# joedownard/skill-chaining-with-graphs

Measured on AMD Instinct MI355X. Metric: env-steps/sec (whole node), 65 536 parallel Pinball envs at 1/2/4/8 MI355X, higher is better.
Workload: dtype f32

## Files before the change

### skill-chaining-with-graphs_amd/csrc/scg_kernels.hip

```cpp
#include "scg_device.hpp"
#include "../../include/scg_abi.h"
#include <cstdio>
#include <cstdlib>
#include <cstring>
#include <cmath>
#include <mutex>
#include <new>
#include <type_traits>
#include <vector>

using namespace scg;
typedef float f4v __attribute__((ext_vector_type(4)));
typedef unsigned u4v __attribute__((ext_vector_type(4)));

#include "scg_eval.hpp"
#include "scg_step_kernel.hpp"
#include "scg_rollout_kernel.hpp"
#include "scg_trial_kernel.hpp"
#include "scg_order.hpp"
#include "scg_collect_kernels.hpp"
#include "scg_reduce_kernel.hpp"
#include "scg_apply_kernels.hpp"
#include "scg_aux_kernels.hpp"

__attribute__((visibility("hidden"))) hipError_t launch_rollout_record(const RolloutRecArgs &A, int grid, hipStream_t s);
__attribute__((visibility("hidden"))) hipError_t launch_trial_record(const TrialRecArgs &A, int grid, hipStream_t s);
__attribute__((visibility("hidden"))) hipError_t launch_rollout_interrupt(const RolloutIntArgs &A, int grid, hipStream_t s);
__attribute__((visibility("hidden"))) hipError_t launch_rollout_interrupt_record(const RolloutIntRecArgs &A, int grid, hipStream_t s);

struct scg_ctx {
    scg_config cfg;
    int n_vf;
    int nblk;
    int n_cu;
    bool have_map;
    MapScalars ms;
    float *d_edges, *d_starts, *d_scale;
    uint64_t *d_cellmask;
    int32_t *d_perm, *d_hist;
    int32_t *d_collect_rows;
    int32_t *d_frontier_rows;
    uint32_t arm_bits;
    const uint8_t *arm_prev;
    const int32_t *arm_count;
    int32_t arm_L;
    bool arm_rows_ready;
    unsigned long long *d_fit_part;
    uint32_t *h_async;
    uint32_t *d_async;
    int32_t *d_fail;
    double fit_timeout_s;
    float4 *d_outrec;
    float4 *d_qalt;
    int32_t *d_invperm;
    int32_t *d_hist2[2];
    int hist_parity;
    bool hist_dirty;
    bool order_valid;
    const int32_t *order_ids;
    uint32_t parents;
    uint32_t gest;
    int32_t *gest_succ;
    float *ring_x, *ring_y;
    uint8_t *events;
    int32_t *ev_len;
    int32_t ring_len;
    unsigned long long *d_stamps;
    float *d_slabs;
    int32_t *d_cnts;
    float *d_G;
    int32_t *d_nk;
    float *G_out;
    int32_t *nk_out;
    float *nkf_out;
    bool prof_on;
    int prof_every;
    long long prof_seen;
    std::vector<hipEvent_t> *prof_ev;
    size_t prof_used;
    char *peer_region;
    size_t peer_bytes, peer_op_stride;
    hipIpcMemHandle_t peer_handle;
    int peer_n, peer_rank;
    char *peer_base[PEER_MAX];
    bool peer_mapped[PEER_MAX];
    uint32_t peer_e;
    int32_t *d_peer_go;
    double peer_timeout_s;
    char err[256];
};

static std::mutex g_peer_mu;
static std::vector<std::pair<hipIpcMemHandle_t, char *>> g_peer_regions;

static thread_local char g_err[256] = "";

#define SCG_HIP(ctx, call)                                                                     \
    do {                                                                                       \
        hipError_t e_ = (call);                                                                \
        if (e_ != hipSuccess) {                                                                \
            snprintf((ctx) ? (ctx)->err : g_err, 256, "%s failed: %s", #call, hipGetErrorString(e_)); \
            return SCG_ERR_HIP;                                                                \
        }                                                                                      \
    } while (0)

static int fail(scg_ctx *ctx, int code, const char *msg) {
    snprintf(ctx ? ctx->err : g_err, 256, "%s", msg);
    return code;
}

static int fail_in(scg_ctx *c, int code, const char *fn, const char *why) {
    char msg[256];
    snprintf(msg, sizeof(msg), "%s: %s", fn, why);
    return fail(c, code, msg);
}

static bool pow2(int x) { return x > 0 && !(x & (x - 1)); }
static bool bad_window(int32_t l_pos, int32_t l_neg) {
    return l_pos < 0 || l_neg < 0 || (int64_t)l_pos + l_neg < 1 || (int64_t)l_pos + l_neg > INT32_MAX;
}

static int decode_async(uint32_t word, char *buf, size_t n) {
    if (word == 0) { if (buf && n) buf[0] = 0; return SCG_OK; }
    if (buf && n) {
        if (word & SCG_ASYNC_STEP_HANDOFF)
            snprintf(buf, n, "an earlier scg_step gave up inside a workgroup: a bounded hand-off poll between its wavefront subsets ran "
                     "out (a logic error or a hung wavefront); the block's partial gradients were dropped and the step's outputs for "
                     "its envs are unspecified — restore the state. scg_clear_async_error() re-arms the context");
        else if (word & SCG_ASYNC_PEER_TIMEOUT)
            snprintf(buf, n, "an earlier scg_peer_exchange_apply gave up: the peer wait ran out (a peer rank did not publish its "
                     "operand within the peer timeout: stopped, hung or out of step); the weights were left unchanged. "
                     "scg_clear_async_error() re-arms the context");
        else if (word & SCG_ASYNC_FIT_TIMEOUT)
            snprintf(buf, n, "an earlier scg_fit_initiation gave up (problem mask 0x%x): its workgroups did not become "
                     "co-resident within the fit timeout (card shared with other work?); the affected classifier rows were "
                     "left unchanged. scg_clear_async_error() re-arms the context", (word >> 8) & 0xffffu);
        else
            snprintf(buf, n, "unknown asynchronous device status 0x%x", word);
    }
    return SCG_ERR_ASYNC;
}
static int async_pending(scg_ctx *c);
#define SCG_CHECK_ASYNC(c) do { if (async_pending(c)) return SCG_ERR_ASYNC; } while (0)

struct DeviceGuard {
    int prev = -1;
    bool ok = true;
    explicit DeviceGuard(int dev) {
        int cur = -1;
        if (hipGetDevice(&cur) != hipSuccess) { ok = false; return; }
        if (cur != dev) {
            if (hipSetDevice(dev) != hipSuccess) { ok = false; return; }
            prev = cur;
        }
    }
    ~DeviceGuard() { if (prev >= 0) (void)hipSetDevice(prev); }
    DeviceGuard(const DeviceGuard &) = delete;
    DeviceGuard &operator=(const DeviceGuard &) = delete;
};
#define SCG_ON_DEVICE(c, what)                                                                   \
    DeviceGuard dev_guard_((c)->cfg.device);                                                     \
    if (!dev_guard_.ok) return fail((c), SCG_ERR_HIP, what ": cannot make the context's device current")

static int async_pending(scg_ctx *c) {
    if (!c || !c->h_async) return 0;
    const uint32_t w = *reinterpret_cast<volatile uint32_t *>(c->h_async);
    if (w == 0) return 0;
    decode_async(w, c->err, sizeof(c->err));
    return 1;
}

extern "C" {

int scg_abi_version(void) { return SCG_ABI_VERSION; }

int scg_decode_async_word(uint32_t word, char *buf, int32_t buf_len) {
    return decode_async(word, buf, buf_len > 0 ? (size_t)buf_len : 0);
}

int scg_async_status(scg_ctx *c, void *stream, int32_t synchronize, uint32_t *word_out) {
    if (!c) return fail(nullptr, SCG_ERR_INVALID, "scg_async_status: null ctx");
    if (synchronize) {
        SCG_ON_DEVICE(c, "scg_async_status");
        SCG_HIP(c, hipStreamSynchronize(reinterpret_cast<hipStream_t>(stream)));
    }
    const uint32_t w = c->h_async ? *reinterpret_cast<volatile uint32_t *>(c->h_async) : 0u;
    if (word_out) *word_out = w;
    return decode_async(w, c->err, sizeof(c->err));
}

int scg_clear_async_error(scg_ctx *c) {
    if (!c) return fail(nullptr, SCG_ERR_INVALID, "scg_clear_async_error: null ctx");
    if (c->h_async) *reinterpret_cast<volatile uint32_t *>(c->h_async) = 0u;
    if (c->d_fail) {
        DeviceGuard g(c->cfg.device);
        if (g.ok) (void)hipMemset(c->d_fail, 0, sizeof(int32_t));
    }
    c->order_valid = false; c->hist_dirty = true; c->arm_rows_ready = false;
    return SCG_OK;
}

static int set_timeout(scg_ctx *c, const char *fn, double scg_ctx::*field, double seconds) {
    if (!c) return fail_in(nullptr, SCG_ERR_INVALID, fn, "null ctx");
    if (!(seconds >= 0.0) || seconds > 3600.0) return fail_in(c, SCG_ERR_INVALID, fn, "seconds must be in [0, 3600]");
    c->*field = seconds;
    return SCG_OK;
}

int scg_set_fit_timeout(scg_ctx *c, double seconds) { return set_timeout(c, "scg_set_fit_timeout", &scg_ctx::fit_timeout_s, seconds); }

int scg_set_peer_timeout(scg_ctx *c, double seconds) { return set_timeout(c, "scg_set_peer_timeout", &scg_ctx::peer_timeout_s, seconds); }

int scg_debug_raise_async(scg_ctx *c, uint32_t word) {
    if (!c || !c->h_async) return fail(c, SCG_ERR_INVALID, "scg_debug_raise_async: null ctx");
    *reinterpret_cast<volatile uint32_t *>(c->h_async) |= word;
    return SCG_OK;
}

int scg_block_envs(void) { return BLOCK_ENVS; }

const char *scg_strerror(int status) {
    switch (status) {
        case SCG_OK: return "ok";
        case SCG_ERR_INVALID: return "invalid argument";
        case SCG_ERR_NO_DEVICE: return "no usable HIP device";
        case SCG_ERR_HIP: return "HIP runtime error";
        case SCG_ERR_STATE: return "call order / state error";
        case SCG_ERR_ASYNC: return "an earlier launch failed on the device";
        default: return "unknown status";
    }
}

const char *scg_last_error(const scg_ctx *ctx) { return ctx ? ctx->err : g_err; }

static size_t hist_bytes(const scg_ctx *c) { return (size_t)((c->cfg.n_envs + 255) / 256) * HSTRIDE * sizeof(int32_t); }

struct CtxAlloc { void **ptr; size_t bytes; bool zero; };
static std::vector<CtxAlloc> ctx_allocs(scg_ctx *c) {
    auto P = [](auto **p) { return reinterpret_cast<void **>(p); };
    const size_t w = (size_t)c->n_vf * NACT * NF * sizeof(float), npos = (size_t)c->nblk * BLOCK_ENVS;
    const size_t rows = (size_t)(c->cfg.n_envs + COL_ROW - 1) / COL_ROW + 1;
    return {
        {P(&c->d_slabs), (size_t)c->nblk * w, false},
        {P(&c->d_cnts), (size_t)c->nblk * c->n_vf * sizeof(int32_t), true},
        {P(&c->d_G), w, true},
        {P(&c->d_nk), MAX_VF * sizeof(int32_t), true},
        {P(&c->d_edges), MAX_EDGES * 8 * sizeof(float), false},
        {P(&c->d_scale), NF * sizeof(float), false},
        {P(&c->d_perm), npos * sizeof(int32_t), false},
        {P(&c->d_hist), hist_bytes(c), false},
        {P(&c->d_collect_rows), rows * sizeof(int32_t), false},
        {P(&c->d_frontier_rows), MAX_VF * rows * sizeof(int32_t), false},
        {P(&c->d_fit_part), (size_t)FIT_BATCH * 2 * FIT_G * 8 * sizeof(unsigned long long), false},
        {P(&c->d_fail), sizeof(int32_t), true},
        {P(&c->d_outrec), npos * OREC * sizeof(float4), false},
        {P(&c->d_qalt), npos * 2 * sizeof(float4), false},
        {P(&c->d_invperm), npos * sizeof(int32_t), false},
        {P(&c->d_hist2[0]), hist_bytes(c), true},
        {P(&c->d_hist2[1]), hist_bytes(c), true},
        {P(&c->d_cellmask), (size_t)CELL_G * CELL_G * 4 * sizeof(uint64_t), false},
    };
}

#ifdef SCG_REDUCE_STAMPS
static size_t reduce_stamp_bytes(const scg_ctx *c) {
    const int nrow = (c->cfg.n_envs + 255) / 256, sy = (nrow + RED_NCOL - 1) / RED_NCOL;
    return (size_t)RED_NCOL * (c->n_vf + sy) * RED_STAMP_SLOTS * sizeof(unsigned long long);
}
#endif

int scg_create(scg_ctx **out, const scg_config *cfg) {
    if (!out || !cfg) return fail(nullptr, SCG_ERR_INVALID, "scg_create: null argument");
    *out = nullptr;
    if (cfg->n_envs < 1) return fail(nullptr, SCG_ERR_INVALID, "scg_create: n_envs must be >= 1");
    if (cfg->n_options < 0 || cfg->n_options > SCG_MAX_OPTIONS)
        return fail(nullptr, SCG_ERR_INVALID, "scg_create: n_options out of range [0,5]");
    if (cfg->update_count_floor < 0) return fail(nullptr, SCG_ERR_INVALID, "scg_create: update_count_floor must be >= 0");
    if (cfg->reoffer_period != 0 && !pow2(cfg->reoffer_period))
        return fail(nullptr, SCG_ERR_INVALID, "scg_create: reoffer_period must be a power of two (or 0)");
    if (cfg->fourier_order != SCG_FOURIER_ORDER)
        return fail(nullptr, SCG_ERR_INVALID, "scg_create: only Fourier order 5 is built");
    int ndev = 0;
    if (hipGetDeviceCount(&ndev) != hipSuccess || ndev < 1)
        return fail(nullptr, SCG_ERR_NO_DEVICE, "scg_create: no HIP device visible");
    if (cfg->device < 0 || cfg->device >= ndev)
        return fail(nullptr, SCG_ERR_INVALID, "scg_create: device ordinal out of range");
    scg_ctx *c = new (std::nothrow) scg_ctx();
    if (!c) return fail(nullptr, SCG_ERR_INVALID, "scg_create: out of host memory");
    memset(c, 0, sizeof(*c));
    c->cfg = *cfg;
    c->n_vf = cfg->n_options + 1;
    c->nblk = (cfg->n_envs + BLOCK_ENVS - 1) / BLOCK_ENVS;
    if (hipDeviceGetAttribute(&c->n_cu, hipDeviceAttributeMultiprocessorCount, cfg->device) != hipSuccess || c->n_cu <= 0) c->n_cu = 256;
    int st = SCG_OK;
    DeviceGuard dev_guard_(cfg->device);
    do {
        if (!dev_guard_.ok) { st = SCG_ERR_HIP; break; }
        for (const CtxAlloc &a : ctx_allocs(c)) {
            if (hipMalloc(a.ptr, a.bytes) != hipSuccess || (a.zero && hipMemset(*a.ptr, 0, a.bytes) != hipSuccess)) { st = SCG_ERR_HIP; break; }
        }
        if (st != SCG_OK) break;
        if (hipHostMalloc(reinterpret_cast<void **>(&c->h_async), 64, hipHostMallocMapped) != hipSuccess) { st = SCG_ERR_HIP; break; }
        *c->h_async = 0u;
        if (hipHostGetDevicePointer(reinterpret_cast<void **>(&c->d_async), c->h_async, 0) != hipSuccess) { st = SCG_ERR_HIP; break; }
    } while (0);
    if (st != SCG_OK) {
        snprintf(g_err, 256, "scg_create: device allocation/setup failed: %s", hipGetErrorString(hipGetLastError()));
        scg_destroy(c);
        return st;
    }
#ifdef SCG_STAMPS_LITE
    if (hipMalloc(&c->d_stamps, (size_t)c->nblk * STAMP_SLOTS * sizeof(unsigned long long)) == hipSuccess)
        (void)hipMemset(c->d_stamps, 0, (size_t)c->nblk * STAMP_SLOTS * sizeof(unsigned long long));
#endif
#ifdef SCG_REDUCE_STAMPS
    if (hipMalloc(&c->d_stamps, reduce_stamp_bytes(c)) == hipSuccess) (void)hipMemset(c->d_stamps, 0, reduce_stamp_bytes(c));
#endif
    c->parents = 0;
    for (int k = 1; k < MAX_VF; ++k) c->parents |= (uint32_t)(k - 1) << (3 * k);
    c->G_out = c->d_G; c->nk_out = c->d_nk;
    c->fit_timeout_s = 2.0;
    c->peer_timeout_s = 2.0;
    *out = c;
    return SCG_OK;
}

int scg_destroy(scg_ctx *c) {
    if (!c) return SCG_OK;
    for (const CtxAlloc &a : ctx_allocs(c)) (void)hipFree(*a.ptr);
    (void)hipFree(c->d_starts);
    if (c->h_async) (void)hipHostFree(c->h_async);
    if (c->peer_region) {
        DeviceGuard g(c->cfg.device);
        for (int r = 0; r < PEER_MAX; ++r)
            if (c->peer_mapped[r]) (void)hipIpcCloseMemHandle(c->peer_base[r]);
        {
            std::lock_guard<std::mutex> lk(g_peer_mu);
            for (size_t i = 0; i < g_peer_regions.size(); ++i)
                if (g_peer_regions[i].second == c->peer_region) { g_peer_regions.erase(g_peer_regions.begin() + i); break; }
        }
        (void)hipFree(c->peer_region); (void)hipFree(c->d_peer_go);
    }
    if (c->prof_ev) {
        for (hipEvent_t e : *c->prof_ev) (void)hipEventDestroy(e);
        delete c->prof_ev;
    }
    delete c;
    return SCG_OK;
}

int scg_set_hparams(scg_ctx *c, float gamma, float alpha, float epsilon, float r_option_success,
                    int32_t max_episode_steps, int32_t max_option_steps, int32_t update_count_floor, int32_t reoffer_period) {
    if (!c) return fail(nullptr, SCG_ERR_INVALID, "scg_set_hparams: null ctx");
    if (update_count_floor < 0) return fail(c, SCG_ERR_INVALID, "scg_set_hparams: update_count_floor must be >= 0");
    if (reoffer_period != 0 && !pow2(reoffer_period)) return fail(c, SCG_ERR_INVALID, "scg_set_hparams: reoffer_period must be a power of two (or 0)");
    c->cfg.gamma = gamma; c->cfg.alpha = alpha; c->cfg.epsilon = epsilon;
    c->cfg.r_option_success = r_option_success;
    c->cfg.max_episode_steps = max_episode_steps; c->cfg.max_option_steps = max_option_steps;
    c->cfg.update_count_floor = update_count_floor;
    c->cfg.reoffer_period = reoffer_period;
    return SCG_OK;
}

int scg_set_map(scg_ctx *c, const float *edges, int32_t n_edges, const float *starts, int32_t n_starts,
                const float map_scalars[6], const float *scale) {
    if (!c) return fail(nullptr, SCG_ERR_INVALID, "scg_set_map: null ctx");
    if (!edges || !starts || !map_scalars || !scale) return fail(c, SCG_ERR_INVALID, "scg_set_map: null argument");
    if (n_edges < 0 || n_edges > MAX_EDGES) return fail(c, SCG_ERR_INVALID, "scg_set_map: n_edges out of range [0,256]");
    if (n_starts < 1) return fail(c, SCG_ERR_INVALID, "scg_set_map: need at least one start position");
    SCG_ON_DEVICE(c, "scg_set_map");
    if (c->d_starts) { (void)hipFree(c->d_starts); c->d_starts = nullptr; }
    SCG_HIP(c, hipMalloc(&c->d_starts, (size_t)n_starts * 2 * sizeof(float)));
    if (n_edges > 0) SCG_HIP(c, hipMemcpy(c->d_edges, edges, (size_t)n_edges * 8 * sizeof(float), hipMemcpyHostToDevice));
    SCG_HIP(c, hipMemcpy(c->d_starts, starts, (size_t)n_starts * 2 * sizeof(float), hipMemcpyHostToDevice));
    SCG_HIP(c, hipMemcpy(c->d_scale, scale, NF * sizeof(float), hipMemcpyHostToDevice));
    const float R = map_scalars[0];
    c->ms.hstep = map_scalars[1]; c->ms.R2 = map_scalars[2];
    c->ms.TX = map_scalars[3]; c->ms.TY = map_scalars[4]; c->ms.TR2 = map_scalars[5];
    c->ms.R = R; c->ms.TR = (float)(std::sqrt((double)map_scalars[5]) * 1.0001);
    {
        std::vector<uint64_t> cm((size_t)CELL_G * CELL_G * 4, 0);
        const double vmax = 2.0 * std::sqrt(2.0) * 1.001;
        const double reach = (double)R * (1.02 + 1.10 * vmax) * 1.01 + 0.5 * std::sqrt(2.0) / CELL_G + 1e-6;
        for (int cy = 0; cy < CELL_G; ++cy)
            for (int cx = 0; cx < CELL_G; ++cx) {
                const double px = (cx + 0.5) / CELL_G, py = (cy + 0.5) / CELL_G;
                for (int j = 0; j < n_edges; ++j) {
                    const float *E = edges + 8 * j;
                    const double dx = px - E[0], dy = py - E[1];
                    double t = (dx * E[2] + dy * E[3]) * E[4];
                    t = t < 0 ? 0 : (t > 1 ? 1 : t);
                    const double qx = E[0] + E[2] * t - px, qy = E[1] + E[3] * t - py;
                    if (std::sqrt(qx * qx + qy * qy) <= reach)
                        cm[((size_t)cy * CELL_G + cx) * 4 + (j >> 6)] |= (1ull << (j & 63));
                }
            }
        SCG_HIP(c, hipMemcpy(c->d_cellmask, cm.data(), cm.size() * sizeof(uint64_t), hipMemcpyHostToDevice));
    }
    c->ms.n_edges = n_edges; c->ms.n_starts = n_starts;
    c->have_map = true;
    return SCG_OK;
}

struct PeerTarget {
    scg_ctx *c;
    float *G, *nkf;
    int32_t *nk;
    explicit PeerTarget(scg_ctx *ctx) : c(ctx), G(ctx->G_out), nkf(ctx->nkf_out), nk(ctx->nk_out) {
        if (!c->peer_n) return;
        float *op = reinterpret_cast<float *>(c->peer_region + PEER_HDR + (c->peer_e & 1u) * c->peer_op_stride);
        c->G_out = op; c->nkf_out = op + (size_t)c->n_vf * NACT * NF; c->nk_out = c->d_nk;
    }
    ~PeerTarget() { c->G_out = G; c->nkf_out = nkf; c->nk_out = nk; }
};

extern "C++" template <typename Args>
static void fill_shared(const scg_ctx *c, Args &A) {
    memset(&A, 0, sizeof(A));
    A.n = c->cfg.n_envs; A.n_vf = c->n_vf;
    A.seed = c->cfg.seed; A.env_base = c->cfg.env_id_base;
    A.epsilon = c->cfg.epsilon; A.max_ep = c->cfg.max_episode_steps; A.max_opt = c->cfg.max_option_steps;
    A.reoffer_mask = c->cfg.reoffer_period > 1 ? (uint32_t)(c->cfg.reoffer_period - 1) : 0u;
    A.parents = c->parents; A.gest = c->gest;
    A.ms = c->ms;
    A.edges = c->d_edges; A.starts = c->d_starts; A.cellmask = c->d_cellmask;
}

static void fill_common(const scg_ctx *c, StepArgs &A) {
    fill_shared(c, A);
    A.gamma = c->cfg.gamma; A.r_succ = c->cfg.r_option_success;
    A.slabs = c->d_slabs; A.cnts = c->d_cnts;
    A.gest_succ = c->gest_succ;
    A.ring_x = c->ring_x; A.ring_y = c->ring_y; A.events = c->events; A.ev_len = c->ev_len;
    A.ring_mask = c->ring_len > 0 ? c->ring_len - 1 : 0;
    A.stamps = c->d_stamps;
    A.async_word = c->d_async; A.fail_flag = c->d_fail;
}

enum ReduceMode { REDUCE_ONLY, COMMIT_ONLY, REDUCE_COMMIT, REDUCE_COMMIT_SORT };
static int launch_reduce(scg_ctx *c, float *W, uint32_t apply, int nblk, hipStream_t s, ReduceMode mode, const StepArgs *st = nullptr) {
    ReduceArgs R;
    memset(&R, 0, sizeof(R));
    R.slabs = c->d_slabs; R.cnts = c->d_cnts; R.G = c->G_out; R.n_k = c->nk_out; R.nk_f = c->nkf_out; R.W = W; R.scale = c->d_scale;
    R.nblk = nblk; R.n_vf = c->n_vf; R.alpha = c->cfg.alpha; R.apply = apply; R.fail_flag = c->d_fail; R.nk_floor = c->cfg.update_count_floor;
    const int nrow = st ? (c->cfg.n_envs + 255) / 256 : 0;
    R.n = c->cfg.n_envs; R.nrow = nrow;
    if (st) {
        R.outrec = c->d_outrec; R.qalt = c->d_qalt; R.invperm = c->d_invperm; R.perm = c->d_perm; R.sort = mode == REDUCE_COMMIT_SORT ? 1 : 0;
        R.hist = c->d_hist2[c->hist_parity]; R.hist_zero = c->d_hist2[c->hist_parity ^ 1];
        R.x = st->x; R.y = st->y; R.vx = st->vx; R.vy = st->vy; R.reward = st->reward;
        R.option_id_out = st->option_id; R.opt_steps = st->opt_steps; R.ep_steps = st->ep_steps;
        R.action = st->action; R.done = st->done;
        R.qcache = st->k_hi >= 0 ? st->qcache : nullptr;
        if (c->arm_bits && c->events && c->ring_x) {
            R.c_events = c->events; R.c_prev = c->arm_prev; R.c_evlen = c->ev_len; R.c_count = c->arm_count;
            R.c_rows = c->d_collect_rows; R.c_bits = c->arm_bits; R.c_L = c->arm_L; R.c_ring_len = c->ring_len;
        }
    }
#ifdef SCG_REDUCE_STAMPS
    R.stamps = c->d_stamps;
#endif
    if (mode == COMMIT_ONLY) {
        hipLaunchKernelGGL(commit_kernel, dim3(nrow), dim3(256), 0, s, R);
        SCG_HIP(c, hipGetLastError());
        return SCG_OK;
    }
    const int sy = (nrow + RED_NCOL - 1) / RED_NCOL;
    if (RED_NCOL * (c->n_vf + sy) <= c->n_cu)
        hipLaunchKernelGGL(reduce_kernel<16>, dim3(RED_NCOL, c->n_vf + sy), dim3(RED_THREADS), 0, s, R);
    else
        hipLaunchKernelGGL(reduce_kernel<8>, dim3(RED_NCOL, c->n_vf + sy), dim3(RED_THREADS), 0, s, R);
    SCG_HIP(c, hipGetLastError());
    return SCG_OK;
}

static int sort_env_order(scg_ctx *c, const int32_t *option_id, hipStream_t s) {
    if (c->order_valid && c->order_ids == option_id) return SCG_OK;
    const int nrow = (c->cfg.n_envs + 255) / 256;
    hipLaunchKernelGGL(sort_hist_kernel, dim3(nrow), dim3(256), 0, s, option_id, c->cfg.n_envs, c->n_vf, c->d_hist);
    hipLaunchKernelGGL(sort_scatter_kernel, dim3(nrow), dim3(256), 0, s, option_id, c->cfg.n_envs, c->n_vf, nrow,
                       c->d_hist, c->d_perm, c->d_invperm);
    SCG_HIP(c, hipGetLastError());
    return SCG_OK;
}

static int prof_begin(scg_ctx *c, hipStream_t s, hipEvent_t &ev1) {
    if (!(c->prof_on && (c->prof_seen++ % c->prof_every) == c->prof_every / 2)) return SCG_OK;
    if (!c->prof_ev) c->prof_ev = new std::vector<hipEvent_t>();
    while (c->prof_ev->size() < c->prof_used + 2) {
        hipEvent_t e;
        SCG_HIP(c, hipEventCreate(&e));
        c->prof_ev->push_back(e);
    }
    hipEvent_t ev0 = (*c->prof_ev)[c->prof_used];
    ev1 = (*c->prof_ev)[c->prof_used + 1];
    c->prof_used += 2;
    SCG_HIP(c, hipEventRecord(ev0, s));
    return SCG_OK;
}

int scg_step(scg_ctx *c, float *x, float *y, float *vx, float *vy, int32_t *option_id, int32_t *opt_steps,
             int32_t *ep_steps, float *qcache, uint8_t *action, float *reward, uint8_t *done, float *W,
             const float *clf, uint32_t enabled_mask, uint64_t t, uint32_t flags, void *stream) {
    if (!c) return fail(nullptr, SCG_ERR_INVALID, "scg_step: null ctx");
    if (!c->have_map) return fail(c, SCG_ERR_STATE, "scg_step: scg_set_map has not been called");
    if (!x || !y || !vx || !vy || !option_id || !opt_steps || !ep_steps || !qcache || !action || !reward ||
        !done || !W || !clf)
        return fail(c, SCG_ERR_INVALID, "scg_step: null array argument");
    if (c->peer_n && (flags & SCG_STEP_LEARN) && (flags & SCG_STEP_APPLY))
        return fail(c, SCG_ERR_INVALID, "scg_step: SCG_STEP_APPLY with a peer region open (the update is scg_peer_exchange_apply's)");
    if ((flags & SCG_STEP_INTERRUPT) && !(flags & SCG_STEP_LEARN))
        return fail(c, SCG_ERR_INVALID, "scg_step: SCG_STEP_INTERRUPT without SCG_STEP_LEARN (acting-only interruption is scg_rollout_interrupt)");
    SCG_CHECK_ASYNC(c);
    SCG_ON_DEVICE(c, "scg_step");
    if (c->arm_bits) {
        const void *ptrs[2] = {c->arm_count, c->arm_prev};
        for (const void *p : ptrs) {
            if (!p) continue;
            hipPointerAttribute_t at;
            if (hipPointerGetAttributes(&at, p) != hipSuccess || at.type != hipMemoryTypeDevice) {
                (void)hipGetLastError();
                c->arm_bits = 0; c->arm_rows_ready = false;
                return fail(c, SCG_ERR_STATE, "scg_step: the buffers announced with scg_arm_collect are no longer device memory "
                                              "(freed before scg_arm_collect(0)?); the trigger has been disarmed");
            }
        }
    }
    hipStream_t s = reinterpret_cast<hipStream_t>(stream);
    StepArgs A;
    fill_common(c, A);
    A.x = x; A.y = y; A.vx = vx; A.vy = vy;
    A.option_id = option_id; A.opt_steps = opt_steps; A.ep_steps = ep_steps; A.qcache = qcache;
    A.action = action; A.reward = reward; A.done = done;
    A.W = W; A.clf = clf;
    A.k_lo = 0; A.k_hi = c->n_vf - 1;
    A.enabled = enabled_mask; A.learn = (flags & SCG_STEP_LEARN) ? 1u : 0u; A.t = t;
    if (flags & 0x100u) A.k_hi = -1;
    if (const int rc = sort_env_order(c, option_id, s)) return rc;
    c->order_valid = false;
    if (c->hist_dirty) {
        const size_t hb = hist_bytes(c);
        SCG_HIP(c, hipMemsetAsync(c->d_hist2[0], 0, hb, s));
        SCG_HIP(c, hipMemsetAsync(c->d_hist2[1], 0, hb, s));
        c->hist_dirty = false;
    }
    const bool fold = (flags & SCG_STEP_LEARN) && !(flags & 0x200u);
    A.hist_next = fold ? c->d_hist2[c->hist_parity] : nullptr;
    A.perm = c->d_perm; A.outrec = c->d_outrec; A.qalt = c->d_qalt;
    hipEvent_t ev1 = nullptr;
    if (const int rc = prof_begin(c, s, ev1)) return rc;
    if (flags & SCG_STEP_INTERRUPT)
        hipLaunchKernelGGL(td_kernel<MODE_FUSED_INT>, dim3(c->nblk), dim3(THREADS), 0, s, A);
    else
        hipLaunchKernelGGL(td_kernel<MODE_FUSED>, dim3(c->nblk), dim3(THREADS), 0, s, A);
    SCG_HIP(c, hipGetLastError());
    if (ev1) SCG_HIP(c, hipEventRecord(ev1, s));
    c->arm_rows_ready = c->arm_bits && c->events && c->ring_x;
    if (!(flags & SCG_STEP_LEARN)) return launch_reduce(c, W, 0u, c->nblk, s, COMMIT_ONLY, &A);
    PeerTarget peer_target(c);
    if (!fold) return launch_reduce(c, W, (flags & SCG_STEP_APPLY) ? 1u : 0u, c->nblk, s, REDUCE_COMMIT, &A);
    c->hist_dirty = true;
    const int rc = launch_reduce(c, W, (flags & SCG_STEP_APPLY) ? 1u : 0u, c->nblk, s, REDUCE_COMMIT_SORT, &A);
    if (rc != SCG_OK) return rc;
    c->hist_dirty = false;
    c->hist_parity ^= 1;
    c->order_valid = true; c->order_ids = option_id;
    return SCG_OK;
}

static bool rollout_epw(const scg_ctx *c, int n, int &epw) {
    epw = 2;
    while (epw < RO_MAX_EPW && (long long)n >= (long long)c->n_cu * RO_WAVES * epw * 2) epw *= 2;
    if (const char *ov = getenv("SCG_ROLLOUT_EPW")) {
        const int v = atoi(ov);
        if (v < 2 || v > RO_MAX_EPW || !pow2(v)) return false;
        epw = v;
    }
    return true;
}

static int check_record(scg_ctx *c, const char *fn, const scg_record *rec, int N, long long min_rows) {
    const char *why = !rec->len ? "rec->len is required" : rec->n < 1 ? "rec->n must be >= 1"
                    : rec->first < 0 || (long long)rec->first + rec->n > N ? "rec->first .. first+n-1 outside the envs / entries"
                    : rec->rows < min_rows ? "rec->rows too small for the launch's pseudo-steps" : nullptr;
    return why ? fail_in(c, SCG_ERR_INVALID, fn, why) : SCG_OK;
}

extern "C++" template <typename Derived, typename Base, typename Set>
static Derived derived_args(const Base &base, Set set) {
    Derived D;
    memset(&D, 0, sizeof(D));
    static_cast<Base &>(D) = base;
    set(D);
    return D;
}

static int rollout_launch(const char *fn, scg_ctx *c, float *x, float *y, float *vx, float *vy, int32_t *option_id, int32_t *opt_steps,
                          int32_t *ep_steps, float *qcache, uint8_t *action, float *reward, uint8_t *done,
                          const float *W, const float *clf, uint32_t enabled_mask, uint64_t t0, int32_t n_steps,
                          uint32_t flags, const scg_rollout_stats *stats, const scg_record *rec, bool at, void *stream,
                          bool intr = false, int32_t *interrupts = nullptr) {
    if (!c) return fail_in(nullptr, SCG_ERR_INVALID, fn, "null ctx");
    if (!c->have_map) return fail_in(c, SCG_ERR_STATE, fn, "scg_set_map has not been called");
    if (!x || !y || !vx || !vy || !option_id || !opt_steps || !ep_steps || !qcache || !action || !reward ||
        !done || !W || !clf)
        return fail_in(c, SCG_ERR_INVALID, fn, "null array argument");
    if (flags & ~(SCG_ROLLOUT_BEGIN | SCG_ROLLOUT_ONE_EPISODE)) return fail_in(c, SCG_ERR_INVALID, fn, "unknown flag");
    if (n_steps < 0 || n_steps > SCG_ROLLOUT_MAX_STEPS)
        return fail_in(c, SCG_ERR_INVALID, fn, "n_steps out of range [0, SCG_ROLLOUT_MAX_STEPS]");
    if (n_steps == 0 && !(flags & SCG_ROLLOUT_BEGIN))
        return fail_in(c, SCG_ERR_INVALID, fn, "n_steps == 0 without SCG_ROLLOUT_BEGIN (or _BEGIN_AT)");
    if ((flags & SCG_ROLLOUT_ONE_EPISODE) && !(stats && stats->finished))
        return fail_in(c, SCG_ERR_INVALID, fn, "SCG_ROLLOUT_ONE_EPISODE needs stats->finished");
    if (rec) {
        const int rc = check_record(c, fn, rec, c->cfg.n_envs, (long long)n_steps + ((flags & SCG_ROLLOUT_BEGIN) ? 1 : 0));
        if (rc != SCG_OK) return rc;
    }
    SCG_CHECK_ASYNC(c);
    DeviceGuard dev_guard_(c->cfg.device);
    if (!dev_guard_.ok) return fail_in(c, SCG_ERR_HIP, fn, "cannot make the context's device current");
    RolloutArgs R;
    fill_shared(c, R);
    R.x = x; R.y = y; R.vx = vx; R.vy = vy; R.option_id = option_id; R.opt_steps = opt_steps; R.ep_steps = ep_steps;
    R.qcache = qcache; R.action = action; R.reward = reward; R.done = done; R.W = W; R.clf = clf;
    if (stats) R.st = *stats;
    R.n_steps = n_steps;
    R.begin = (flags & SCG_ROLLOUT_BEGIN) ? 1u : 0u; R.one_episode = (flags & SCG_ROLLOUT_ONE_EPISODE) ? 1u : 0u;
    R.enabled = enabled_mask; R.t0 = t0;
    int epw;
    if (!rollout_epw(c, c->cfg.n_envs, epw)) return fail_in(c, SCG_ERR_INVALID, fn, "SCG_ROLLOUT_EPW must be 2, 4, 8, 16 or 32");
    R.epw = epw;
    const int grid = (c->cfg.n_envs + RO_WAVES * epw - 1) / (RO_WAVES * epw);
    c->order_valid = false;
    if (intr && (rec || at)) {
        const auto RR = derived_args<RolloutIntRecArgs>(R, [&](auto &D) { if (rec) D.rec = *rec; D.begin_at = at ? 1u : 0u; D.interrupts = interrupts; });
        SCG_HIP(c, launch_rollout_interrupt_record(RR, grid, reinterpret_cast<hipStream_t>(stream)));
    } else if (intr) {
        const auto RI = derived_args<RolloutIntArgs>(R, [&](auto &D) { D.interrupts = interrupts; });
        SCG_HIP(c, launch_rollout_interrupt(RI, grid, reinterpret_cast<hipStream_t>(stream)));
    } else if (rec || at) {
        const auto RR = derived_args<RolloutRecArgs>(R, [&](auto &D) { if (rec) D.rec = *rec; D.begin_at = at ? 1u : 0u; });
        SCG_HIP(c, launch_rollout_record(RR, grid, reinterpret_cast<hipStream_t>(stream)));
    } else {
        hipLaunchKernelGGL((rollout_kernel<false, RolloutArgs>), dim3(grid), dim3(RO_THREADS), 0, reinterpret_cast<hipStream_t>(stream), R);
        SCG_HIP(c, hipGetLastError());
    }
    return SCG_OK;
}

int scg_rollout(scg_ctx *c, float *x, float *y, float *vx, float *vy, int32_t *option_id, int32_t *opt_steps,
                int32_t *ep_steps, float *qcache, uint8_t *action, float *reward, uint8_t *done,
                const float *W, const float *clf, uint32_t enabled_mask, uint64_t t0, int32_t n_steps,
                uint32_t flags, const scg_rollout_stats *stats, void *stream) {
    return rollout_launch("scg_rollout", c, x, y, vx, vy, option_id, opt_steps, ep_steps, qcache, action, reward, done, W, clf,
                          enabled_mask, t0, n_steps, flags, stats, nullptr, false, stream);
}

static int begin_at_flags(scg_ctx *c, const char *fn, uint32_t &flags, bool &at) {
    at = (flags & SCG_ROLLOUT_BEGIN_AT) != 0;
    if (c && at && (flags & SCG_ROLLOUT_BEGIN))
        return fail_in(c, SCG_ERR_INVALID, fn, "SCG_ROLLOUT_BEGIN and SCG_ROLLOUT_BEGIN_AT together");
    if (at) flags = (flags & ~SCG_ROLLOUT_BEGIN_AT) | SCG_ROLLOUT_BEGIN;
    return SCG_OK;
}

int scg_rollout_record(scg_ctx *c, float *x, float *y, float *vx, float *vy, int32_t *option_id, int32_t *opt_steps,
                       int32_t *ep_steps, float *qcache, uint8_t *action, float *reward, uint8_t *done,
                       const float *W, const float *clf, uint32_t enabled_mask, uint64_t t0, int32_t n_steps,
                       uint32_t flags, const scg_rollout_stats *stats, const scg_record *rec, void *stream) {
    bool at;
    if (const int rc = begin_at_flags(c, "scg_rollout_record", flags, at)) return rc;
    return rollout_launch("scg_rollout_record", c, x, y, vx, vy, option_id, opt_steps, ep_steps, qcache, action, reward, done,
                          W, clf, enabled_mask, t0, n_steps, flags, stats, rec, at, stream);
}

int scg_rollout_interrupt(scg_ctx *c, float *x, float *y, float *vx, float *vy, int32_t *option_id, int32_t *opt_steps,
                          int32_t *ep_steps, float *qcache, uint8_t *action, float *reward, uint8_t *done,
                          const float *W, const float *clf, uint32_t enabled_mask, uint64_t t0, int32_t n_steps,
                          uint32_t flags, const scg_rollout_stats *stats, int32_t *interrupts, const scg_record *rec,
                          void *stream) {
    bool at;
    if (const int rc = begin_at_flags(c, "scg_rollout_interrupt", flags, at)) return rc;
    return rollout_launch("scg_rollout_interrupt", c, x, y, vx, vy, option_id, opt_steps, ep_steps, qcache, action, reward, done,
                          W, clf, enabled_mask, t0, n_steps, flags, stats, rec, at, stream, true, interrupts);
}

static int trials_launch(const char *fn, scg_ctx *c, int32_t n, const float *x, const float *y, const float *vx, const float *vy,
                         const int32_t *option, const float *W, const float *clf, uint32_t enabled_mask, uint64_t t0,
                         const scg_trial_out *out, const scg_record *rec, void *stream) {
    if (!c) return fail_in(nullptr, SCG_ERR_INVALID, fn, "null ctx");
    if (!c->have_map) return fail_in(c, SCG_ERR_STATE, fn, "scg_set_map has not been called");
    if (!x || !y || !vx || !vy || !option || !W || !clf || !out || !out->outcome)
        return fail_in(c, SCG_ERR_INVALID, fn, "null array argument (or out->outcome)");
    if (n < 1) return fail_in(c, SCG_ERR_INVALID, fn, "n must be >= 1");
    if (std::min(c->cfg.max_option_steps, c->cfg.max_episode_steps) > SCG_TRIAL_MAX_STEPS)
        return fail_in(c, SCG_ERR_INVALID, fn, "min(max_option_steps, max_episode_steps) exceeds SCG_TRIAL_MAX_STEPS");
    if (rec) {
        const int rc = check_record(c, fn, rec, n, 1);
        if (rc != SCG_OK) return rc;
    }
    SCG_CHECK_ASYNC(c);
    DeviceGuard dev_guard_(c->cfg.device);
    if (!dev_guard_.ok) return fail_in(c, SCG_ERR_HIP, fn, "cannot make the context's device current");
    TrialArgs T;
    fill_shared(c, T);
    T.n = n;
    T.x = x; T.y = y; T.vx = vx; T.vy = vy; T.option = option; T.out = *out; T.W = W; T.clf = clf;
    T.enabled = enabled_mask; T.t0 = t0;
    T.gamma = c->cfg.gamma; T.r_succ = c->cfg.r_option_success;
    int epw;
    if (!rollout_epw(c, n, epw)) return fail_in(c, SCG_ERR_INVALID, fn, "SCG_ROLLOUT_EPW must be 2, 4, 8, 16 or 32");
    T.epw = epw;
    const int grid = (int)(((long long)n + RO_WAVES * epw - 1) / (RO_WAVES * epw));
    if (rec) {
        const auto TR = derived_args<TrialRecArgs>(T, [&](auto &D) { D.rec = *rec; });
        SCG_HIP(c, launch_trial_record(TR, grid, reinterpret_cast<hipStream_t>(stream)));
    } else {
        hipLaunchKernelGGL((trial_kernel<false, TrialArgs>), dim3(grid), dim3(RO_THREADS), 0, reinterpret_cast<hipStream_t>(stream), T);
        SCG_HIP(c, hipGetLastError());
    }
    return SCG_OK;
}

int scg_option_trials(scg_ctx *c, int32_t n, const float *x, const float *y, const float *vx, const float *vy,
                      const int32_t *option, const float *W, const float *clf, uint32_t enabled_mask, uint64_t t0,
                      const scg_trial_out *out, void *stream) {
    return trials_launch("scg_option_trials", c, n, x, y, vx, vy, option, W, clf, enabled_mask, t0, out, nullptr, stream);
}

int scg_option_trials_record(scg_ctx *c, int32_t n, const float *x, const float *y, const float *vx, const float *vy,
                             const int32_t *option, const float *W, const float *clf, uint32_t enabled_mask, uint64_t t0,
                             const scg_trial_out *out, const scg_record *rec, void *stream) {
    return trials_launch("scg_option_trials_record", c, n, x, y, vx, vy, option, W, clf, enabled_mask, t0, out, rec, stream);
}

int scg_invalidate_order(scg_ctx *c) {
    if (!c) return fail(nullptr, SCG_ERR_INVALID, "scg_invalidate_order: null ctx");
    c->order_valid = false;
    return SCG_OK;
}

#ifdef SCG_STAMPS_LITE
extern "C" int scg_diag_stamps(scg_ctx *c, unsigned long long *host_out , int32_t reset) {
    if (!c || !c->d_stamps) return SCG_ERR_STATE;
    if (host_out && hipMemcpy(host_out, c->d_stamps, (size_t)c->nblk * STAMP_SLOTS * sizeof(unsigned long long), hipMemcpyDeviceToHost) != hipSuccess) return SCG_ERR_HIP;
    if (reset) (void)hipMemset(c->d_stamps, 0, (size_t)c->nblk * STAMP_SLOTS * sizeof(unsigned long long));
    return SCG_OK;
}
#endif

#ifdef SCG_REDUCE_STAMPS
extern "C" int scg_diag_reduce_stamps(scg_ctx *c, unsigned long long *host_out, int32_t reset) {
    if (!c || !c->d_stamps) return -1;
    if (host_out && hipMemcpy(host_out, c->d_stamps, reduce_stamp_bytes(c), hipMemcpyDeviceToHost) != hipSuccess) return -1;
    if (reset) (void)hipMemset(c->d_stamps, 0, reduce_stamp_bytes(c));
    return (int)(reduce_stamp_bytes(c) / (RED_STAMP_SLOTS * sizeof(unsigned long long)));
}
#endif

int scg_set_option_parents(scg_ctx *c, const int32_t *parents) {
    if (!c || !parents) return fail(c, SCG_ERR_INVALID, "scg_set_option_parents: null argument");
    uint32_t packed = 0;
    for (int k = 1; k <= c->cfg.n_options; ++k) {
        if (parents[k] < 0 || parents[k] > c->cfg.n_options || parents[k] == k)
            return fail(c, SCG_ERR_INVALID, "scg_set_option_parents: parent must be 0 (goal) or another option");
        packed |= (uint32_t)parents[k] << (3 * k);
    }
    for (int k = 1; k <= c->cfg.n_options; ++k) {
        int p = k, hops = 0;
        while (p != 0 && hops <= SCG_MAX_OPTIONS) { p = parents[p]; ++hops; }
        if (p != 0) return fail(c, SCG_ERR_INVALID, "scg_set_option_parents: the option graph has a cycle");
    }
    c->parents = packed;
    return SCG_OK;
// ... 399 lines not shown
```

### skill-chaining-with-graphs_amd/csrc/scg_reduce_kernel.hpp

```cpp
#pragma once

struct ReduceArgs {
    const float *slabs;
    const int32_t *cnts;
    float *G;
    int32_t *n_k;
    float *nk_f;
    float *W;
    const float *scale;
    int32_t nblk, n_vf;
    float alpha;
    uint32_t apply;
    int32_t nk_floor;
    const int32_t *option_id;
    int32_t *hist, *hist_zero, *perm;
    int32_t n, nrow;
    const float4 *outrec;
    const float4 *qalt;
    int32_t *invperm;
    float *x, *y, *vx, *vy, *reward;
    int32_t *option_id_out, *opt_steps, *ep_steps;
    uint8_t *action, *done;
    float *qcache;
    int32_t sort;
    const int32_t *fail_flag;
    const uint8_t *c_events, *c_prev;
    const int32_t *c_evlen, *c_count;
    int32_t *c_rows;
    uint32_t c_bits;
    int32_t c_L, c_ring_len;
#ifdef SCG_REDUCE_STAMPS
    unsigned long long *stamps;
#endif
};

constexpr int SEG = 16;
constexpr int RED_WAVES = 16;
constexpr int RED_THREADS = 64 * RED_WAVES;
constexpr int RED_SPW = 2;
constexpr int RED_COLS = NACT * NF / 4;
constexpr int RED_NCOL = (RED_COLS + 63) / 64;
constexpr int RED_STAMP_SLOTS = 8;

__device__ __forceinline__ void commit_and_place_row(const ReduceArgs &R, int row, int wv, int lane, int (*s_x)[40]) {
    int zoff = 0;
    asm volatile("" : "+v"(zoff));
    const int step_failed = R.fail_flag[zoff];
    const bool act = wv < 4 && row < R.nrow;
    const int e = row * 256 + wv * 64 + lane;
    const bool ok = act && e < R.n;
    const int pos_old = ok ? R.invperm[e] : 0;
    int tot[NKEY], pre[NKEY];
#pragma unroll
    for (int k = 0; k < NKEY; ++k) { tot[k] = 0; pre[k] = 0; }
    if (act && R.sort) {
        for (int r = wv * 64 + lane; r < R.nrow; r += 256) {
#pragma unroll
            for (int k = 0; k < NKEY; ++k) {
                const int h = R.hist[r * HSTRIDE + k];
                tot[k] += h;
                if (r < row) pre[k] += h;
            }
        }
    }
    float4 ra = make_float4(0.0f, 0.0f, 0.0f, 0.0f), rb = ra, rq = ra;
    float q4 = 0.0f;
    if (ok) {
        const float4 *r = R.outrec + (size_t)pos_old * OREC;
        const float4 r3 = r[3];
        ra = r[0]; rb = r[1]; rq = r[2]; q4 = r3.x;
        if (__float_as_uint(r3.y) == OREC_DECLINED) {
            rq = R.qalt[(size_t)pos_old * 2]; q4 = R.qalt[(size_t)pos_old * 2 + 1].x;
            rb.y = __uint_as_float(__float_as_uint(rb.y) | 0x01000000u);
        }
    }
    int key = -1;
    uint64_t km[NKEY];
    if (act) {
        if (R.sort) {
#pragma unroll
            for (int k = 0; k < NKEY; ++k) {
#pragma unroll
                for (int m = 1; m < 64; m <<= 1) { tot[k] += __shfl_xor(tot[k], m, 64); pre[k] += __shfl_xor(pre[k], m, 64); }
            }
        }
        const unsigned bits = __float_as_uint(rb.y);
        if (ok && !step_failed) {
            const int on = (int)((bits >> 16) & 255u);
            const bool declined = (bits >> 24) & 1u;
            const int oid = declined ? -on : (on ? on : -(int)((bits >> 28) & 7u));
            key = sort_key(oid, R.n_vf);
            R.x[e] = ra.x; R.y[e] = ra.y; R.vx[e] = ra.z; R.vy[e] = ra.w;
            R.reward[e] = rb.x; R.action[e] = (uint8_t)(bits & 255u); R.done[e] = (uint8_t)((bits >> 8) & 255u);
            R.option_id_out[e] = oid; R.opt_steps[e] = __float_as_int(rb.z); R.ep_steps[e] = __float_as_int(rb.w);
            if (R.qcache) {
                const size_t n = (size_t)R.n;
                R.qcache[e] = rq.x; R.qcache[n + e] = rq.y; R.qcache[2 * n + e] = rq.z;
                R.qcache[3 * n + e] = rq.w; R.qcache[4 * n + e] = q4;
            }
        }
        if (R.sort) {
#pragma unroll
            for (int k = 0; k < NKEY; ++k) km[k] = __ballot(key == k);
            if (lane < 3 * NKEY) {
                int v = 0;
#pragma unroll
                for (int k = 0; k < NKEY; ++k) {
                    if (lane == k) v = tot[k];
                    if (lane == NKEY + k) v = pre[k];
                    if (lane == 2 * NKEY + k) v = __popcll(km[k]);
                }
                s_x[wv][lane] = v;
            }
        }
    }
    if (R.c_rows && act) {
        bool in;
        int v = collect_v(e, R.n, R.c_events, R.c_prev, R.c_bits, R.c_evlen, R.c_ring_len, R.c_L, in);
#pragma unroll
        for (int m = 1; m < 64; m <<= 1) v += __shfl_xor(v, m, 64);
        if (lane == 0) s_x[wv][3 * NKEY] = v;
    }
    if (!R.sort && !R.c_rows) return;
    __syncthreads();
    if (R.c_rows && wv == 0 && lane == 0 && row < R.nrow) {
        R.c_rows[row] = s_x[0][3 * NKEY] + s_x[1][3 * NKEY] + s_x[2][3 * NKEY] + s_x[3][3 * NKEY];
        if (row == 0) R.c_rows[R.nrow] = *R.c_count;
    }
    if (!R.sort || !act) return;
    int off[NKEY];
#pragma unroll
    for (int k = 0; k < NKEY; ++k) {
        tot[k] = s_x[0][k] + s_x[1][k] + s_x[2][k] + s_x[3][k];
        off[k] = s_x[0][NKEY + k] + s_x[1][NKEY + k] + s_x[2][NKEY + k] + s_x[3][NKEY + k];
#pragma unroll
        for (int w = 0; w < 3; ++w) off[k] += w < wv ? s_x[w][2 * NKEY + k] : 0;
    }
    OrderLayout L;
    order_layout(tot, R.n, L);
    int rk = -1, st = 0;
#pragma unroll
    for (int k = 0; k < NKEY; ++k)
        if (key == k) { rk = off[k] + __popcll(km[k] & ((1ull << lane) - 1ull)); st = L.start[k]; }
    if (rk >= 0 && !step_failed) {
        const int pos = key == 0 ? order_pos0(L, rk) : order_posk(L, st, rk);
        R.perm[pos] = e; R.invperm[e] = pos;
    }
    if (wv == 0 && lane < HSTRIDE) R.hist_zero[row * HSTRIDE + lane] = 0;
}

__device__ __forceinline__ int lane_now() {
    int ln;
    asm volatile("v_mbcnt_lo_u32_b32 %0, -1, 0\n\tv_mbcnt_hi_u32_b32 %0, -1, %0" : "=v"(ln));
    return ln;
}

__device__ __forceinline__ int row_sum(int v) {
    v += __builtin_amdgcn_mov_dpp(v, 0xB1, 0xF, 0xF, true);
    v += __builtin_amdgcn_mov_dpp(v, 0x4E, 0xF, 0xF, true);
    v += __builtin_amdgcn_mov_dpp(v, 0x141, 0xF, 0xF, true);
    v += __builtin_amdgcn_mov_dpp(v, 0x140, 0xF, 0xF, true);
    return v;
}

#ifdef SCG_REDUCE_STAMPS
#define RED_STAMP(slot) do { \
        if (R.stamps && lane_now() == 0) \
            R.stamps[(size_t)__builtin_amdgcn_readfirstlane((int)(blockIdx.y * gridDim.x + blockIdx.x) * RED_STAMP_SLOTS + (slot))] = __builtin_amdgcn_s_memrealtime(); \
    } while (0)
#define RED_STAMP_DRAINED(slot) do { asm volatile("s_waitcnt vmcnt(0) lgkmcnt(0)" ::: "memory"); RED_STAMP(slot); } while (0)
#else
#define RED_STAMP(slot) do { } while (0)
#define RED_STAMP_DRAINED(slot) do { } while (0)
#endif

template <int BATCH>
__global__ __launch_bounds__(RED_THREADS, BATCH == 16 ? 4 : 8) void reduce_kernel(const ReduceArgs R) {
    __shared__ float4 s_T[RED_WAVES * RED_SPW][64];
    __shared__ int s_cnt[RED_WAVES * RED_SPW];
    __shared__ int s_x[4][40];
    const int sy_rows = (int)gridDim.y - R.n_vf;
    const int wave = __builtin_amdgcn_readfirstlane((int)threadIdx.x >> 6);
    RED_STAMP(0);
    if ((int)blockIdx.y < sy_rows) {
        const int row = (int)blockIdx.y * (int)gridDim.x + blockIdx.x;
        commit_and_place_row(R, row, wave, threadIdx.x & 63, s_x);
        if (wave < 4) RED_STAMP_DRAINED(1 + wave);
        return;
    }
    const int k = (int)blockIdx.y - sy_rows;
    const size_t slab_stride = (size_t)R.n_vf * RED_COLS * sizeof(float4);
    const char *slab_k = reinterpret_cast<const char *>(R.slabs) + (size_t)k * RED_COLS * sizeof(float4);
    const int nseg = (R.nblk + SEG - 1) / SEG;
    float4 S = make_float4(0.0f, 0.0f, 0.0f, 0.0f);
    int nk = 0;
    float4 w_old = make_float4(0.0f, 0.0f, 0.0f, 0.0f), sc = w_old;
    int step_failed = 0;
    for (int sg0 = 0; sg0 < nseg; sg0 += RED_WAVES * RED_SPW) {
        const int lane = lane_now();
        int cs[RED_SPW];
#pragma unroll
        for (int j = 0; j < RED_SPW; ++j) {
            const int bl = (sg0 + j * RED_WAVES + wave) * SEG + (lane & (SEG - 1));
            cs[j] = R.cnts[(unsigned)(min(bl, R.nblk - 1) * R.n_vf + k)];
        }
#pragma unroll
        for (int j = 0; j < RED_SPW; ++j) {
            const int b0 = (sg0 + j * RED_WAVES + wave) * SEG;
            const int c = (lane < SEG && b0 + lane < R.nblk) ? cs[j] : 0;
            const unsigned mask = (unsigned)__ballot(c > 0);
            float4 T = make_float4(0.0f, 0.0f, 0.0f, 0.0f);
            if (mask) {
                const __amdgpu_buffer_rsrc_t seg = __builtin_amdgcn_make_buffer_rsrc(
                    const_cast<char *>(slab_k + (size_t)b0 * slab_stride), 0, 0x7fffffff, 0x00020000);
                const int i4 = blockIdx.x * 64 + lane;
                const unsigned col_off = (unsigned)(i4 < RED_COLS ? i4 : 0) * (unsigned)sizeof(float4);
#pragma unroll
                for (int h = 0; h < SEG; h += BATCH) {
                    if (!((mask >> h) & ((1u << BATCH) - 1u))) continue;
                    u4v v[BATCH];
#pragma unroll
                    for (int u = 0; u < BATCH; ++u) {
                        v[u] = (u4v){0u, 0u, 0u, 0u};
                        if ((mask >> (h + u)) & 1u) v[u] = __builtin_amdgcn_raw_buffer_load_b128(seg, (int)col_off, (int)((h + u) * (unsigned)slab_stride), 0);
                    }
#pragma unroll
                    for (int u = 0; u < BATCH; ++u) {
                        if ((mask >> (h + u)) & 1u) {
                            T.x = T.x + __uint_as_float(v[u][0]); T.y = T.y + __uint_as_float(v[u][1]);
                            T.z = T.z + __uint_as_float(v[u][2]); T.w = T.w + __uint_as_float(v[u][3]);
                        }
                    }
                }
            }
            __builtin_amdgcn_s_waitcnt(0x0F70);
            s_T[j * RED_WAVES + wave][lane] = T;
            const int ctot = row_sum(c);
            if (lane == 0) s_cnt[j * RED_WAVES + wave] = ctot;
        }
        const bool last = sg0 + RED_WAVES * RED_SPW >= nseg;
        if (wave == 0 && last) RED_STAMP(5);
        if (wave == 0 && R.apply && last) {
            step_failed = *R.fail_flag;
            const int i4 = blockIdx.x * 64 + lane_now();
            const int col = i4 < RED_COLS ? i4 : 0;
            w_old = reinterpret_cast<const float4 *>(R.W)[(size_t)k * RED_COLS + col];
            sc = *reinterpret_cast<const float4 *>(R.scale + (col * 4) % NF);
        }
        __syncthreads();
        if (wave == 0) {
            if (last) RED_STAMP(6);
            const int ln = lane_now();
            const int cu = row_sum(ln < RED_WAVES * RED_SPW ? s_cnt[ln] : 0);
            nk += __builtin_amdgcn_readlane(cu, 0) + __builtin_amdgcn_readlane(cu, 16);
#pragma unroll
            for (int h = 0; h < RED_WAVES * RED_SPW; h += BATCH) {
                float4 t[BATCH];
#pragma unroll
                for (int u = 0; u < BATCH; ++u) t[u] = s_T[h + u][ln];
#pragma unroll
                for (int u = 0; u < BATCH; ++u) { S.x = S.x + t[u].x; S.y = S.y + t[u].y; S.z = S.z + t[u].z; S.w = S.w + t[u].w; }
            }
            if (last) RED_STAMP(7);
        }
        if (!last) __syncthreads();
    }
    if (wave != 0) return;
    const int lane = lane_now(), i4 = blockIdx.x * 64 + lane;
    if (blockIdx.x == 0 && lane == 0) {
        R.n_k[k] = nk;
        if (R.nk_f) R.nk_f[k] = (float)nk;
    }
    if (i4 >= RED_COLS) return;
    reinterpret_cast<float4 *>(R.G)[(size_t)k * RED_COLS + i4] = S;
    if (R.apply && nk > 0 && !step_failed) {
        const float step = R.alpha / (float)max(nk, R.nk_floor);
        float4 w = w_old;
        w.x = fmaf(step * sc.x, S.x, w.x); w.y = fmaf(step * sc.y, S.y, w.y);
        w.z = fmaf(step * sc.z, S.z, w.z); w.w = fmaf(step * sc.w, S.w, w.w);
        reinterpret_cast<float4 *>(R.W)[(size_t)k * RED_COLS + i4] = w;
    }
    RED_STAMP_DRAINED(1);
}

__global__ __launch_bounds__(256) void commit_kernel(const ReduceArgs R) {
    __shared__ int s_x[4][40];
    commit_and_place_row(R, blockIdx.x, threadIdx.x >> 6, threadIdx.x & 63, s_x);
}
```

Baseline: 884.7 million.

## Split root option reduction across two blocks with unconditional prefetched slab loads

Option k=0 (the root, likely carrying most envs) is now reduced by RED_ROOT_SPLIT blocks, each covering half the columns, which adds one grid row. For k=0 the per-segment loads are issued unconditionally in a software-pipelined ring, and non-contributing blocks are masked out in the accumulate step rather than by branching. The final shared-memory sum also stops early past the last valid segment. This aims to shorten the critical-path block of the reduce kernel, at the cost of a larger grid that may fall back to the BATCH=8 variant, and of redundant loads for blocks with zero counts.

```diff
diff --git a/skill-chaining-with-graphs_amd/csrc/scg_kernels.hip b/skill-chaining-with-graphs_amd/csrc/scg_kernels.hip
--- a/skill-chaining-with-graphs_amd/csrc/scg_kernels.hip
+++ b/skill-chaining-with-graphs_amd/csrc/scg_kernels.hip
@@ -265,7 +265,7 @@
 #ifdef SCG_REDUCE_STAMPS
 static size_t reduce_stamp_bytes(const scg_ctx *c) {
     const int nrow = (c->cfg.n_envs + 255) / 256, sy = (nrow + RED_NCOL - 1) / RED_NCOL;
-    return (size_t)RED_NCOL * (c->n_vf + sy) * RED_STAMP_SLOTS * sizeof(unsigned long long);
+    return (size_t)RED_NCOL * (c->n_vf + RED_ROOT_SPLIT - 1 + sy) * RED_STAMP_SLOTS * sizeof(unsigned long long);
 }
 #endif
 
@@ -465,11 +465,11 @@
         SCG_HIP(c, hipGetLastError());
         return SCG_OK;
     }
-    const int sy = (nrow + RED_NCOL - 1) / RED_NCOL;
-    if (RED_NCOL * (c->n_vf + sy) <= c->n_cu)
-        hipLaunchKernelGGL(reduce_kernel<16>, dim3(RED_NCOL, c->n_vf + sy), dim3(RED_THREADS), 0, s, R);
+    const int sy = (nrow + RED_NCOL - 1) / RED_NCOL, gy = sy + RED_ROOT_SPLIT - 1 + c->n_vf;
+    if (RED_NCOL * gy <= c->n_cu)
+        hipLaunchKernelGGL(reduce_kernel<16>, dim3(RED_NCOL, gy), dim3(RED_THREADS), 0, s, R);
     else
-        hipLaunchKernelGGL(reduce_kernel<8>, dim3(RED_NCOL, c->n_vf + sy), dim3(RED_THREADS), 0, s, R);
+        hipLaunchKernelGGL(reduce_kernel<8>, dim3(RED_NCOL, gy), dim3(RED_THREADS), 0, s, R);
     SCG_HIP(c, hipGetLastError());
     return SCG_OK;
 }
diff --git a/skill-chaining-with-graphs_amd/csrc/scg_reduce_kernel.hpp b/skill-chaining-with-graphs_amd/csrc/scg_reduce_kernel.hpp
--- a/skill-chaining-with-graphs_amd/csrc/scg_reduce_kernel.hpp
+++ b/skill-chaining-with-graphs_amd/csrc/scg_reduce_kernel.hpp
@@ -40,6 +40,7 @@
 constexpr int RED_SPW = 2;
 constexpr int RED_COLS = NACT * NF / 4;
 constexpr int RED_NCOL = (RED_COLS + 63) / 64;
+constexpr int RED_ROOT_SPLIT = 2;
 constexpr int RED_STAMP_SLOTS = 8;
 
 __device__ __forceinline__ void commit_and_place_row(const ReduceArgs &R, int row, int wv, int lane, int (*s_x)[40]) {
@@ -149,6 +150,11 @@
     if (wv == 0 && lane < HSTRIDE) R.hist_zero[row * HSTRIDE + lane] = 0;
 }
 
+__device__ __forceinline__ int red_col(int ln, int part, int lw) {
+    const int i4 = (int)blockIdx.x * 64 + part * lw + ln;
+    return (ln < lw && i4 < RED_COLS) ? i4 : -1;
+}
+
 __device__ __forceinline__ int lane_now() {
     int ln;
     asm volatile("v_mbcnt_lo_u32_b32 %0, -1, 0\n\tv_mbcnt_hi_u32_b32 %0, -1, %0" : "=v"(ln));
@@ -179,7 +185,7 @@
     __shared__ float4 s_T[RED_WAVES * RED_SPW][64];
     __shared__ int s_cnt[RED_WAVES * RED_SPW];
     __shared__ int s_x[4][40];
-    const int sy_rows = (int)gridDim.y - R.n_vf;
+    const int sy_rows = (int)gridDim.y - R.n_vf - (RED_ROOT_SPLIT - 1);
     const int wave = __builtin_amdgcn_readfirstlane((int)threadIdx.x >> 6);
     RED_STAMP(0);
     if ((int)blockIdx.y < sy_rows) {
@@ -188,7 +194,9 @@
         if (wave < 4) RED_STAMP_DRAINED(1 + wave);
         return;
     }
-    const int k = (int)blockIdx.y - sy_rows;
+    const int ks = (int)blockIdx.y - sy_rows;
+    const int k = max(ks - (RED_ROOT_SPLIT - 1), 0);
+    const int part = k == 0 ? ks : 0, lw = k == 0 ? 64 / RED_ROOT_SPLIT : 64;
     const size_t slab_stride = (size_t)R.n_vf * RED_COLS * sizeof(float4);
     const char *slab_k = reinterpret_cast<const char *>(R.slabs) + (size_t)k * RED_COLS * sizeof(float4);
     const int nseg = (R.nblk + SEG - 1) / SEG;
@@ -207,28 +215,54 @@
 #pragma unroll
         for (int j = 0; j < RED_SPW; ++j) {
             const int b0 = (sg0 + j * RED_WAVES + wave) * SEG;
-            const int c = (lane < SEG && b0 + lane < R.nblk) ? cs[j] : 0;
-            const unsigned mask = (unsigned)__ballot(c > 0);
             float4 T = make_float4(0.0f, 0.0f, 0.0f, 0.0f);
-            if (mask) {
-                const __amdgpu_buffer_rsrc_t seg = __builtin_amdgcn_make_buffer_rsrc(
-                    const_cast<char *>(slab_k + (size_t)b0 * slab_stride), 0, 0x7fffffff, 0x00020000);
-                const int i4 = blockIdx.x * 64 + lane;
-                const unsigned col_off = (unsigned)(i4 < RED_COLS ? i4 : 0) * (unsigned)sizeof(float4);
-#pragma unroll
-                for (int h = 0; h < SEG; h += BATCH) {
-                    if (!((mask >> h) & ((1u << BATCH) - 1u))) continue;
+            int c = 0;
+            if (k == 0) {
+                if (b0 < R.nblk && lane < lw) {
+                    const __amdgpu_buffer_rsrc_t seg = __builtin_amdgcn_make_buffer_rsrc(
+                        const_cast<char *>(slab_k + (size_t)b0 * slab_stride), 0, 0x7fffffff, 0x00020000);
+                    const int i4 = red_col(lane, part, lw);
+                    const unsigned col_off = (unsigned)(i4 >= 0 ? i4 : 0) * (unsigned)sizeof(float4);
+                    const int ulast = min(SEG, R.nblk - b0) - 1;
                     u4v v[BATCH];
 #pragma unroll
-                    for (int u = 0; u < BATCH; ++u) {
-                        v[u] = (u4v){0u, 0u, 0u, 0u};
-                        if ((mask >> (h + u)) & 1u) v[u] = __builtin_amdgcn_raw_buffer_load_b128(seg, (int)col_off, (int)((h + u) * (unsigned)slab_stride), 0);
+                    for (int u = 0; u < BATCH; ++u)
+                        v[u] = __builtin_amdgcn_raw_buffer_load_b128(seg, (int)col_off, (int)((unsigned)min(u, ulast) * (unsigned)slab_stride), 0);
+                    c = (lane < SEG && b0 + lane < R.nblk) ? cs[j] : 0;
+                    const unsigned mask = (unsigned)__ballot(c > 0);
+#pragma unroll
+                    for (int u = 0; u < SEG; ++u) {
+                        const bool has = (mask >> u) & 1u;
+                        const u4v w = v[u % BATCH];
+                        T.x = T.x + (has ? __uint_as_float(w[0]) : 0.0f); T.y = T.y + (has ? __uint_as_float(w[1]) : 0.0f);
+                        T.z = T.z + (has ? __uint_as_float(w[2]) : 0.0f); T.w = T.w + (has ? __uint_as_float(w[3]) : 0.0f);
+                        if (u + BATCH < SEG)
+                            v[u % BATCH] = __builtin_amdgcn_raw_buffer_load_b128(seg, (int)col_off, (int)((unsigned)min(u + BATCH, ulast) * (unsigned)slab_stride), 0);
                     }
-#pragma unroll
-                    for (int u = 0; u < BATCH; ++u) {
-                        if ((mask >> (h + u)) & 1u) {
-                            T.x = T.x + __uint_as_float(v[u][0]); T.y = T.y + __uint_as_float(v[u][1]);
-                            T.z = T.z + __uint_as_float(v[u][2]); T.w = T.w + __uint_as_float(v[u][3]);
+                }
+            } else {
+                c = (lane < SEG && b0 + lane < R.nblk) ? cs[j] : 0;
+                const unsigned mask = (unsigned)__ballot(c > 0);
+                if (mask) {
+                    const __amdgpu_buffer_rsrc_t seg = __builtin_amdgcn_make_buffer_rsrc(
+                        const_cast<char *>(slab_k + (size_t)b0 * slab_stride), 0, 0x7fffffff, 0x00020000);
+                    const int i4 = blockIdx.x * 64 + lane;
+                    const unsigned col_off = (unsigned)(i4 < RED_COLS ? i4 : 0) * (unsigned)sizeof(float4);
+#pragma unroll
+                    for (int h = 0; h < SEG; h += BATCH) {
+                        if (!((mask >> h) & ((1u << BATCH) - 1u))) continue;
+                        u4v v[BATCH];
+#pragma unroll
+                        for (int u = 0; u < BATCH; ++u) {
+                            v[u] = (u4v){0u, 0u, 0u, 0u};
+                            if ((mask >> (h + u)) & 1u) v[u] = __builtin_amdgcn_raw_buffer_load_b128(seg, (int)col_off, (int)((h + u) * (unsigned)slab_stride), 0);
+                        }
+#pragma unroll
+                        for (int u = 0; u < BATCH; ++u) {
+                            if ((mask >> (h + u)) & 1u) {
+                                T.x = T.x + __uint_as_float(v[u][0]); T.y = T.y + __uint_as_float(v[u][1]);
+                                T.z = T.z + __uint_as_float(v[u][2]); T.w = T.w + __uint_as_float(v[u][3]);
+                            }
                         }
                     }
                 }
@@ -242,8 +276,8 @@
         if (wave == 0 && last) RED_STAMP(5);
         if (wave == 0 && R.apply && last) {
             step_failed = *R.fail_flag;
-            const int i4 = blockIdx.x * 64 + lane_now();
-            const int col = i4 < RED_COLS ? i4 : 0;
+            const int i4 = red_col(lane_now(), part, lw);
+            const int col = i4 >= 0 ? i4 : 0;
             w_old = reinterpret_cast<const float4 *>(R.W)[(size_t)k * RED_COLS + col];
             sc = *reinterpret_cast<const float4 *>(R.scale + (col * 4) % NF);
         }
@@ -255,6 +289,7 @@
             nk += __builtin_amdgcn_readlane(cu, 0) + __builtin_amdgcn_readlane(cu, 16);
 #pragma unroll
             for (int h = 0; h < RED_WAVES * RED_SPW; h += BATCH) {
+                if (h && sg0 + h >= nseg) break;
                 float4 t[BATCH];
 #pragma unroll
                 for (int u = 0; u < BATCH; ++u) t[u] = s_T[h + u][ln];
@@ -266,12 +301,12 @@
         if (!last) __syncthreads();
     }
     if (wave != 0) return;
-    const int lane = lane_now(), i4 = blockIdx.x * 64 + lane;
-    if (blockIdx.x == 0 && lane == 0) {
+    const int lane = lane_now(), i4 = red_col(lane, part, lw);
+    if (blockIdx.x == 0 && part == 0 && lane == 0) {
         R.n_k[k] = nk;
         if (R.nk_f) R.nk_f[k] = (float)nk;
     }
-    if (i4 >= RED_COLS) return;
+    if (i4 < 0) return;
     reinterpret_cast<float4 *>(R.G)[(size_t)k * RED_COLS + i4] = S;
     if (R.apply && nk > 0 && !step_failed) {
         const float step = R.alpha / (float)max(nk, R.nk_floor);
```

Result: no change. 890.5 million, median of 6 (+0.7%).
